# AbeelLab/phasm

Hardware: AMD Instinct MI355X
Metric: overlaps_per_sec (higher is better)
Workload: dtype u64

## Files before the change

phasm_amd/csrc/c_api.hip:

```cpp
#include "../../include/phasm_overlap.h"

#include <hip/hip_runtime.h>

#include <dlfcn.h>
#include <execinfo.h>
#include <fcntl.h>
#include <signal.h>
#include <sys/mman.h>
#include <sys/stat.h>
#include <unistd.h>

#include <algorithm>
#include <array>
#include <atomic>
#include <chrono>
#include <cmath>
#include <condition_variable>
#include <cstdio>
#include <cstdlib>
#include <cstring>
#include <deque>
#include <functional>
#include <memory>
#include <mutex>
// ... 526 lines not shown
}

bool kit_give(po_handle* h) {
    if (getenv("PHASM_NO_KIT_POOL") || !h->stream || !h->copy_stream || !h->up_stream || !h->rc_stream || !h->pinned) return false;
    if (hipStreamSynchronize(h->stream) != hipSuccess || hipStreamSynchronize(h->copy_stream) != hipSuccess ||
        hipStreamSynchronize(h->up_stream) != hipSuccess || hipStreamSynchronize(h->rc_stream) != hipSuccess) {
        (void)hipGetLastError();
        return false;
    }
    DevKit k;
    k.device = h->device;
    k.stream = h->stream;
    k.copy_stream = h->copy_stream;
    k.up_stream = h->up_stream;
    k.rc_stream = h->rc_stream;
    std::memcpy(k.ev_sets, h->ev_sets, sizeof(k.ev_sets));
    k.ev_up0 = h->ev_up0;
    k.ev_up1 = h->ev_up1;
    k.ev_meta = h->ev_meta;
    k.ev_first = h->ev_first;
    std::memcpy(k.ev_piece, h->ev_piece, sizeof(k.ev_piece));
    std::memcpy(k.ev_rc, h->ev_rc, sizeof(k.ev_rc));
    std::memcpy(k.ev_lay, h->ev_lay, sizeof(k.ev_lay));
    k.pinned = h->pinned;
    k.pinned_dev = h->pinned_dev;
    std::lock_guard<std::mutex> lock(g_kit_mu);
    if (g_kits.size() >= KIT_POOL_MAX) return false;
    g_kits.push_back(k);
    return true;
}


unsigned cpu_share() {
    static const unsigned share = [] {
        unsigned n = std::thread::hardware_concurrency();
        n = n ? n : 4u;
        long long q = -1, per = 100000;
        if (FILE* f = std::fopen("/sys/fs/cgroup/cpu.max", "r")) {
            char buf[64] = {0};
            if (std::fscanf(f, "%63s %lld", buf, &per) >= 1 && std::strcmp(buf, "max") != 0) q = atoll(buf);
            std::fclose(f);
        } else if (FILE* g = std::fopen("/sys/fs/cgroup/cpu/cpu.cfs_quota_us", "r")) {
            if (std::fscanf(g, "%lld", &q) != 1) q = -1;
            std::fclose(g);
            if (FILE* g2 = std::fopen("/sys/fs/cgroup/cpu/cpu.cfs_period_us", "r")) {
                if (std::fscanf(g2, "%lld", &per) != 1) per = 100000;
                std::fclose(g2);
            }
        }
        if (q > 0 && per > 0) n = std::min<unsigned>(n, (unsigned)std::max<long long>(1, q / per));
        return n;
    }();
    return share;
}

namespace home {

constexpr uint32_t CHUNK = 4096;

struct Job {
    const void* rec = nullptr;
    uint32_t sh_b = 0, sh_p = 0;
    uint64_t n_rec = 0;
    po_row* out = nullptr;
    uint64_t n_rows = 0;
    const volatile uint32_t* flag = nullptr;
    uint32_t want = 0;
    uint32_t paired = 0, bits = 2;
};

struct Pool {
    std::vector<std::thread> thr;
    std::mutex mu;
    std::condition_variable cv_queue;
    std::condition_variable cv_job;
    std::mutex call_mu;
    std::deque<Job> queue;
    std::atomic<uint64_t> submitted{0}, finished{0};
    std::atomic<int> error{0};
    const uint32_t* len = nullptr;
    uint32_t n_reads = 0;
    std::atomic<uint64_t> sum_l{0}, sum_b{0}, sum_e{0};
    Job cur;
    uint64_t job_seq = 0;
    uint32_t n_chunks = 0;
    std::vector<uint64_t> chunk_off;
    std::atomic<uint32_t> next_count{0}, done_count{0}, next_write{0}, done_write{0};
    std::atomic<int> phase{0};
    std::atomic<int> inside{0};
    std::chrono::steady_clock::time_point t0;
    std::vector<std::array<double, 3>> trace;
    bool tracing = false;
};

Pool* g_pool = nullptr;
std::once_flag g_pool_once;

inline void cpu_pause() {
#if defined(__x86_64__) || defined(__i386__)
    __builtin_ia32_pause();
#endif
}

std::atomic<uint32_t> g_spin_limit{4096};
template <class Pred>
inline void spin_until(Pred pred) {
    const uint32_t limit = g_spin_limit.load(std::memory_order_relaxed);
    for (uint32_t n = 0; !pred(); ++n) {
        if (limit == 0 || n < limit) cpu_pause();
        else std::this_thread::yield();
    }
}

inline po::Cand load_rec(const Job& j, uint64_t i) {
    if (!j.sh_b) return static_cast<const po::Cand*>(j.rec)[i];
    return po::unpack_record(static_cast<const uint64_t*>(j.rec)[i], j.sh_b, j.sh_p);
}

inline uint32_t rows_of_rec(const po::Cand& c, uint32_t paired) {
    if (!paired) return (c.type & 1u) + ((c.type >> 1) & 1u);
    return ((c.type & 1u) ? (c.a == (c.b ^ 1u) ? 1u : 2u) : 0u) + ((c.type & 2u) ? 2u : 0u);
}

inline void put_row(uint64_t*& o, uint32_t a, uint32_t b, uint32_t astart, uint32_t aend, uint32_t bend) {
    __builtin_nontemporal_store((uint64_t)a | ((uint64_t)b << 32), o);
    __builtin_nontemporal_store((uint64_t)astart | ((uint64_t)aend << 32), o + 1);
    __builtin_nontemporal_store((uint64_t)bend << 32, o + 2);
    o += 3;
}

bool expand_records(Pool& P, uint64_t lo, uint64_t hi, po_row* out) {
    uint64_t* o = reinterpret_cast<uint64_t*>(out);
    const Job& job = P.cur;
    const uint32_t* len = P.len;
    const uint32_t paired = job.paired, n_reads = P.n_reads, bits = job.bits;
    auto pb = [bits](uint32_t l) -> uint64_t { return bits == 8u ? l : (l >> 2) + ((l & 3u) != 0u); };
    uint64_t sl = 0, sb = 0, se = 0;
    for (uint64_t i = lo; i < hi; ++i) {
        const po::Cand c = load_rec(job, i);
        if (c.a >= n_reads || c.b >= n_reads) return false;
        const uint32_t la = len[c.a], lb = len[c.b];
        se += 2 * pb((c.type & 1u) ? la - c.p : lb);
        if (c.type & 1u) {
            const uint32_t l = la - c.p;
            const bool twin = paired && c.a != (c.b ^ 1u);
            put_row(o, c.a, c.b, c.p, la, l);
            if (twin) put_row(o, c.b ^ 1u, c.a ^ 1u, lb - l, lb, l);
            const uint64_t k = twin ? 2 : 1;
            sl += k * l;
            sb += k * 2 * pb(l);
        }
        if (c.type & 2u) {
            put_row(o, c.a, c.b, c.p, c.p + lb, lb);
            if (paired) put_row(o, c.a ^ 1u, c.b ^ 1u, la - c.p - lb, la - c.p, lb);
            const uint64_t k = paired ? 2 : 1;
            sl += k * lb;
            sb += k * 2 * pb(lb);
        }
    }
    P.sum_l.fetch_add(sl, std::memory_order_relaxed);
    P.sum_b.fetch_add(sb, std::memory_order_relaxed);
    P.sum_e.fetch_add(se, std::memory_order_relaxed);
    return true;
}

void run_phases(Pool& P, bool lead) {
    const uint32_t nc = P.n_chunks;
    for (;;) {
        const uint32_t c = P.next_count.fetch_add(1, std::memory_order_relaxed);
        if (c >= nc) break;
        const uint64_t lo = (uint64_t)c * CHUNK, hi = std::min<uint64_t>(P.cur.n_rec, lo + CHUNK);
        uint64_t n = 0;
        const uint32_t paired = P.cur.paired;
        for (uint64_t i = lo; i < hi; ++i) n += rows_of_rec(load_rec(P.cur, i), paired);
        P.chunk_off[c + 1] = n;
        P.done_count.fetch_add(1, std::memory_order_release);
    }
    if (lead) {
        spin_until([&] { return P.done_count.load(std::memory_order_acquire) >= nc; });
        P.chunk_off[0] = 0;
        for (uint32_t c = 0; c < nc; ++c) P.chunk_off[c + 1] += P.chunk_off[c];
        if (P.chunk_off[nc] != P.cur.n_rows) P.error.store(1);
        P.phase.store(P.error.load() ? 0 : 2, std::memory_order_release);
    } else {
        spin_until([&] { return P.phase.load(std::memory_order_acquire) != 1; });
    }
    if (P.phase.load(std::memory_order_acquire) != 2) return;
    for (;;) {
        const uint32_t c = P.next_write.fetch_add(1, std::memory_order_relaxed);
        if (c >= nc) break;
        const uint64_t lo = (uint64_t)c * CHUNK, hi = std::min<uint64_t>(P.cur.n_rec, lo + CHUNK);
        if (!expand_records(P, lo, hi, P.cur.out + P.chunk_off[c])) P.error.store(2);
#if defined(__x86_64__)
        __builtin_ia32_sfence();
#endif
        P.done_write.fetch_add(1, std::memory_order_release);
    }
}

void helper(Pool* Pp) {
    Pool& P = *Pp;
    uint64_t seen = 0;
    for (;;) {
        {
            std::unique_lock<std::mutex> lock(P.mu);
            P.cv_job.wait(lock, [&] { return P.job_seq != seen; });
            seen = P.job_seq;
        }
        P.inside.fetch_add(1, std::memory_order_acq_rel);
        if (P.phase.load(std::memory_order_acquire) != 0) run_phases(P, false);
        P.inside.fetch_sub(1, std::memory_order_release);
    }
}

void leader(Pool* Pp) {
    Pool& P = *Pp;
    for (;;) {
        Job j;
        {
            std::unique_lock<std::mutex> lock(P.mu);
            P.cv_queue.wait(lock, [&] { return !P.queue.empty(); });
            j = P.queue.front();
            P.queue.pop_front();
        }
        if (j.flag)
            spin_until([&] { return *j.flag == j.want; });
        std::atomic_thread_fence(std::memory_order_acquire);
        const double t_ready = P.tracing ? std::chrono::duration<double, std::micro>(std::chrono::steady_clock::now() - P.t0).count() : 0.0;
        if (P.error.load() == 0 && j.n_rec) {
            spin_until([&] { return P.inside.load(std::memory_order_acquire) == 0; });
            P.cur = j;
            P.n_chunks = (uint32_t)((j.n_rec + CHUNK - 1) / CHUNK);
            if (P.chunk_off.size() < (size_t)P.n_chunks + 1) P.chunk_off.resize((size_t)P.n_chunks + 1);
            P.next_count.store(0);
            P.done_count.store(0);
            P.next_write.store(0);
            P.done_write.store(0);
            P.phase.store(1, std::memory_order_release);
            {
                std::lock_guard<std::mutex> lock(P.mu);
                ++P.job_seq;
            }
            P.cv_job.notify_all();
            run_phases(P, true);
            if (P.phase.load() == 2)
                spin_until([&] { return P.done_write.load(std::memory_order_acquire) >= P.n_chunks; });
            P.phase.store(0, std::memory_order_release);
            std::atomic_thread_fence(std::memory_order_seq_cst);
        }
        if (P.tracing)
            P.trace.push_back({t_ready, std::chrono::duration<double, std::micro>(std::chrono::steady_clock::now() - P.t0).count(), (double)j.n_rows});
        P.finished.fetch_add(1, std::memory_order_release);
    }
}

Pool* pool() {
    std::call_once(g_pool_once, [] {
        Pool* P = new Pool();
        unsigned n = cpu_share();
        n = std::max(1u, std::min(n * 3 / 4, 12u));
        if (const char* e = getenv("PHASM_HOME_THREADS")) n = (unsigned)std::max(1, std::min(64, atoi(e)));
        try {
            P->thr.emplace_back(leader, P);
            P->thr.back().detach();
            for (unsigned i = 1; i < n; ++i) {
                P->thr.emplace_back(helper, P);
                P->thr.back().detach();
            }
        } catch (const std::system_error&) {
        }
        if (P->thr.empty()) {
            delete P;
            P = nullptr;
        }
        g_pool = P;
    });
    return g_pool;
}

void begin(Pool* P, const uint32_t* len, uint32_t n_reads, bool tracing) {
    if (const char* e = getenv("PHASM_HOME_SPIN")) g_spin_limit.store((uint32_t)std::max(0, atoi(e)));
    else g_spin_limit.store(4096);
    P->len = len;
    P->n_reads = n_reads;
    P->error.store(0);
    P->submitted.store(0);
    P->finished.store(0);
    P->sum_l.store(0);
    P->sum_b.store(0);
    P->sum_e.store(0);
    P->tracing = tracing;
    P->trace.clear();
    P->t0 = std::chrono::steady_clock::now();
}

void submit(Pool* P, const Job& j) {
    {
        std::lock_guard<std::mutex> lock(P->mu);
        P->queue.push_back(j);
    }
    P->submitted.fetch_add(1, std::memory_order_release);
    P->cv_queue.notify_one();
}

void wait_all(Pool* P) {
    spin_until([&] { return P->finished.load(std::memory_order_acquire) >= P->submitted.load(std::memory_order_acquire); });
}

}

po_status init_device(po_handle* h) {
    if (h->dev_ready) {
        HIP_TRY(h, hipSetDevice(h->device));
        return PO_OK;
    }
    AllocTrace tr("init_device", 0);
    const auto ti0 = std::chrono::steady_clock::now();
    auto imark = [&](const char* what) {
        if (tr.on) std::fprintf(stderr, "[init] %s at %.1f ms\n", what, std::chrono::duration<double, std::milli>(std::chrono::steady_clock::now() - ti0).count());
    };
    int n = 0;
    hipError_t e = hipGetDeviceCount(&n);
    imark("runtime up (hipGetDeviceCount)");
    if (e != hipSuccess || n == 0)
        return fail(h, PO_ERR_HIP, "no HIP device available (libphasm_overlap has no CPU fallback)");
    if (h->device < 0 || h->device >= n) return fail(h, PO_ERR_INVALID, "device ordinal out of range");
    HIP_TRY(h, hipSetDevice(h->device));
    hipDeviceProp_t prop;
    HIP_TRY(h, hipGetDeviceProperties(&prop, h->device));
    h->n_cu = prop.multiProcessorCount > 0 ? prop.multiProcessorCount : 256;
    h->lds_max = prop.sharedMemPerBlock;
    if (const char* e = getenv("PHASM_POISON")) h->poison = (int)(strtol(e, nullptr, 0) & 0xFF);
    if (!getenv("PHASM_NO_KIT_POOL") && kit_take(h)) {
        h->ev = h->ev_sets[0];
        std::memset(h->pinned, 0, 1024);
        hipLaunchKernelGGL(po::k_fill_u32, dim3(1), dim3(64), 0, h->stream, reinterpret_cast<uint32_t*>(h->pinned_dev + 63), (uint64_t)1, 0u);
        (void)hipGetLastError();
        h->dev_ready = true;
        return PO_OK;
    }
    imark("device selected, properties read");
    HIP_TRY(h, hipStreamCreateWithFlags(&h->stream, hipStreamNonBlocking));
    imark("first stream made");
    for (int i = 0; i < 2 * EV_N; ++i) HIP_TRY(h, hipEventCreate(&h->ev_sets[i / EV_N][i % EV_N]));
    HIP_TRY(h, hipEventCreate(&h->ev_up0));
    HIP_TRY(h, hipEventCreate(&h->ev_up1));
    imark("first events made");
    HIP_TRY(h, hipHostMalloc(reinterpret_cast<void**>(&h->pinned), 1024, hipHostMallocDefault));
    pin_note(h->pinned, 1024, 1u);
    HIP_TRY(h, hipHostGetDevicePointer(reinterpret_cast<void**>(&h->pinned_dev), h->pinned, 0));
    imark("landing zone made");
    if (const char* e = getenv("PHASM_POISON")) h->poison = (int)(strtol(e, nullptr, 0) & 0xFF);
    HIP_TRY(h, hipStreamCreateWithFlags(&h->copy_stream, hipStreamNonBlocking));
    imark("copy stream made");
    HIP_TRY(h, hipStreamCreateWithFlags(&h->up_stream, hipStreamNonBlocking));
    HIP_TRY(h, hipStreamCreateWithFlags(&h->rc_stream, hipStreamNonBlocking));
    imark("other streams made");
    for (int k = 0; k < PO_MAX_PIECES; ++k) {
        HIP_TRY(h, hipEventCreate(&h->ev_piece[k]));
        HIP_TRY(h, hipEventCreateWithFlags(&h->ev_rc[k], hipEventDisableTiming));
    }
    HIP_TRY(h, hipEventCreateWithFlags(&h->ev_first, hipEventDisableTiming));
    HIP_TRY(h, hipEventCreateWithFlags(&h->ev_meta, hipEventDisableTiming));
    imark("streams and events made");
    hipLaunchKernelGGL(po::k_fill_u32, dim3(1), dim3(64), 0, h->stream, reinterpret_cast<uint32_t*>(h->pinned_dev + 63), (uint64_t)1, 0u);
    (void)hipGetLastError();
    imark("first launch queued (code object loaded)");
    if (!getenv("PHASM_NO_WARM")) {
        void* w = nullptr;
        if (hipMalloc(&w, 256) == hipSuccess) {
            uint32_t* wd = static_cast<uint32_t*>(w);
            (void)hipMemcpyAsync(wd, h->pinned + 62, 8, hipMemcpyHostToDevice, h->up_stream);
            hipLaunchKernelGGL(po::k_fill_u32, dim3(1), dim3(64), 0, h->up_stream, wd + 8, (uint64_t)1, 0u);
            (void)hipMemcpyAsync(wd + 16, h->pinned + 62, 8, hipMemcpyHostToDevice, h->stream);
            hipLaunchKernelGGL(po::k_fill_u32, dim3(1), dim3(64), 0, h->rc_stream, wd + 24, (uint64_t)1, 0u);
            hipLaunchKernelGGL(po::k_fill_u32, dim3(1), dim3(64), 0, h->copy_stream, wd + 32, (uint64_t)1, 0u);
            (void)hipMemcpyAsync(h->pinned + 61, wd + 32, 8, hipMemcpyDeviceToHost, h->copy_stream);
// ... 3123 lines not shown
    *out = nullptr;
    if (h->segments_only) return fail(h, PO_ERR_INVALID, "this handle holds GFA segments without sequences");
    po_result* r = new (std::nothrow) po_result();
    if (!r) return fail(h, PO_ERR_NOMEM, "out of host memory");
    r->h = h;
    po_status st;
    try {
        st = upload(h);
        if (st == PO_OK) st = run_expand(h, candidates_device, n_candidates, r);
    } catch (const std::bad_alloc&) {
        st = fail(h, PO_ERR_NOMEM, "out of host memory in po_expand");
    }
    if (st != PO_OK) {
        if (h->dev_ready) (void)hipStreamSynchronize(h->stream);
        r->d_rows.release();
        delete r;
        return st;
    }
    ++h->live_results;
    *out = r;
    return PO_OK;
}

po_status po_overlaps(po_handle* h, uint32_t min_length, po_result** out) {
    return po_overlaps_shard(h, min_length, 0, 1, out);
}

extern "C++" {
namespace {

struct HostRows {
    HostBuf hb;
    uint64_t total = 0;
};

bool home_begin(po_handle* h) {
    h->home_on = false;
    if (!home_enabled()) return false;
    home::Pool* P = home::pool();
    if (!P) return false;
    P->call_mu.lock();
    home::begin(P, h->len.data(), (uint32_t)h->len.size(), getenv("PHASM_STREAM_TRACE") != nullptr || getenv("PHASM_HOME_TRACE") != nullptr);
    h->home_on = true;
    h->home_used = 0;
    h->home_seq = 0;
    if (h->home_pack_n != h->len.size() || h->home_pack_bases != h->total_bases) {
        uint32_t longest = 0;
        for (uint32_t l : h->len) longest = std::max(longest, l);
        uint32_t br = 1, bp = 1;
        while ((1ull << br) < (uint64_t)h->len.size()) ++br;
        while ((1ull << bp) < (uint64_t)longest + 1ull) ++bp;
        const bool fits = 2 * br + bp <= 62;
        h->home_pack_b = fits ? br : 0u;
        h->home_pack_p = fits ? 2 * br : 0u;
        h->home_pack_n = h->len.size();
        h->home_pack_bases = h->total_bases;
    }
    const char* pk = getenv("PHASM_HOME_PACK");
    const bool pack = !(pk && atoi(pk) == 0);
    h->home_sh_b = pack ? h->home_pack_b : 0u;
    h->home_sh_p = pack ? h->home_pack_p : 0u;
    return true;
}

void home_wait(po_handle* h) {
    if (h->home_on) home::wait_all(home::g_pool);
}

int home_end(po_handle* h, po_stats* sum = nullptr) {
    if (!h->home_on) return 0;
    home::Pool* P = home::g_pool;
    home::wait_all(P);
    const int err = P->error.load();
    if (sum) {
        sum->sum_overlap_bases += P->sum_l.load();
        sum->verify_bytes_algo += P->sum_b.load();
        sum->verify_bytes_exec += P->sum_e.load();
    }
    if (P->tracing)
        for (size_t i = 0; i < P->trace.size(); ++i)
            std::fprintf(stderr, "[home] piece %zu: records home at %.3f ms, %.0f rows written at %.3f ms (since the call set the pool up)\n", i,
                         P->trace[i][0] * 1e-3, P->trace[i][2], P->trace[i][1] * 1e-3);
    h->home_on = false;
    P->call_mu.unlock();
    return err;
}

po_status rows_room(po_handle* h, HostRows& R, uint64_t nk, uint32_t k, uint32_t n_chunks, double seen_share) {
    const size_t need = (size_t)(R.total + nk) * sizeof(po_row);
    if (need <= R.hb.cap) return PO_OK;
    uint64_t guess = std::max<uint64_t>(h->last_host_rows, (R.total + nk) * n_chunks / (k + 1));
    if (seen_share > 0.0) guess = std::max<uint64_t>(guess, (uint64_t)((double)(R.total + nk) / seen_share * 1.05));
    HostBuf bigger;
    PO_TRY(ensure_host(h, bigger, std::max<size_t>(need, (size_t)(guess + guess / 8) * sizeof(po_row))));
    home_wait(h);
    if (hipStreamSynchronize(h->copy_stream) != hipSuccess) {
        bigger.release();
        return fail(h, PO_ERR_HIP, "copy stream");
    }
    if (R.total) std::memcpy(bigger.p, R.hb.p, (size_t)R.total * sizeof(po_row));
    R.hb.release();
    R.hb = bigger;
    return PO_OK;
}

po_status append_home(po_handle* h, HostRows& R, const DevBuf& dev, uint64_t n_rec, uint64_t nk, uint32_t k, uint32_t n_chunks,
                      double seen_share = 0.0) {
    if (nk == 0) return PO_OK;
    home::Pool* P = home::g_pool;
    PO_TRY(rows_room(h, R, nk, k, n_chunks, seen_share));
    const size_t elem = h->home_sh_b ? sizeof(uint64_t) : sizeof(po::Cand);
    const size_t bytes = (size_t)n_rec * elem;
    constexpr uint64_t N_EV = 32;
    if (h->home_used + bytes > h->home_stage.cap || (h->home_seq && h->home_seq % N_EV == 0)) {
        home_wait(h);
        if (hipStreamSynchronize(h->copy_stream) != hipSuccess) return fail(h, PO_ERR_HIP, "copy stream");
        h->home_used = 0;
        if (bytes > h->home_stage.cap)
            PO_TRY(ensure_host(h, h->home_stage, std::max<size_t>({bytes * 2, (size_t)(h->home_last_bytes + h->home_last_bytes / 8), (size_t)8 << 20})));
    }
    const uint32_t slot = (uint32_t)(h->home_seq % N_EV);
    const uint32_t want = ++h->home_gen;
    char* dst = static_cast<char*>(h->home_stage.p) + h->home_used;
    HIP_TRY(h, hipMemcpyAsync(dst, dev.p, bytes, hipMemcpyDeviceToHost, h->copy_stream));
    hipLaunchKernelGGL(po::k_fill_u32, dim3(1), dim3(64), 0, h->copy_stream, reinterpret_cast<uint32_t*>(h->pinned_dev + 96 + slot), (uint64_t)1, want);
    HIP_TRY(h, hipGetLastError());
    home::Job j;
    j.rec = dst;
    j.sh_b = h->home_sh_b;
    j.sh_p = h->home_sh_p;
    j.n_rec = n_rec;
    j.out = static_cast<po_row*>(R.hb.p) + R.total;
    j.n_rows = nk;
    j.flag = reinterpret_cast<const volatile uint32_t*>(h->pinned + 96 + slot);
    j.want = want;
    j.paired = (h->bits == 2 && h->paired) ? 1u : 0u;
    j.bits = (uint32_t)h->bits;
    home::submit(P, j);
    ++h->home_seq;
    h->home_used += (bytes + 255) & ~size_t(255);
    h->home_last_bytes += bytes;
    R.total += nk;
    return PO_OK;
}

po_status append_rows(po_handle* h, HostRows& R, const DevBuf& dev, uint64_t nk, uint32_t k, uint32_t n_chunks, double seen_share = 0.0) {
    if (nk == 0) return PO_OK;
    PO_TRY(rows_room(h, R, nk, k, n_chunks, seen_share));
    HIP_TRY(h, hipMemcpyAsync(static_cast<char*>(R.hb.p) + (size_t)R.total * sizeof(po_row), dev.p, (size_t)nk * sizeof(po_row),
                              hipMemcpyDeviceToHost, h->copy_stream));
    R.total += nk;
    return PO_OK;
}

void add_stats(po_stats& sum, const po_stats& S) {
    sum.n_candidates += S.n_candidates;
    sum.n_verified += S.n_verified;
    sum.n_rows += S.n_rows;
    sum.sum_overlap_bases += S.sum_overlap_bases;
    sum.verify_bytes_algo += S.verify_bytes_algo;
    sum.verify_bytes_exec += S.verify_bytes_exec;
    sum.n_tiles += S.n_tiles;
    sum.shard_bases += S.shard_bases;
    sum.fused_tail += S.fused_tail;
    sum.tail_fallback += S.tail_fallback;
    sum.n_predicted += S.n_predicted;
// ... 1205 lines not shown
po_status po_result_merged_paths(po_result* r, uint64_t* n_paths, uint64_t* n_members, uint64_t* offsets_out, uint64_t cap_paths,
                                 uint32_t* members_out, int32_t* prefix_out, uint64_t cap_members, int64_t* lengths_out) {
    if (!r || !n_paths || !n_members) return PO_ERR_INVALID;
    *n_paths = *n_members = 0;
    po_handle* h = r->h;
    if (!h) return PO_ERR_INVALID;
    if (!r->merged) return fail(h, PO_ERR_INVALID, "po_result_merged_paths needs a po_layout_merge result");
    const uint64_t K = r->n_merged, m = r->n_members;
    *n_paths = K;
    *n_members = m;
    try {
        (void)hipSetDevice(h->device);
        HIP_TRY(h, hipStreamSynchronize(h->stream));
        if (offsets_out && cap_paths >= K) {
            std::vector<uint32_t> off(K);
            if (K) HIP_TRY(h, hipMemcpy(off.data(), r->d_moff.p, K * 4, hipMemcpyDeviceToHost));
            for (uint64_t k = 0; k < K; ++k) offsets_out[k] = off[k];
            offsets_out[K] = m;
        }
        if (lengths_out && cap_paths >= K && K) HIP_TRY(h, hipMemcpy(lengths_out, r->d_mlen.p, K * 8, hipMemcpyDeviceToHost));
        if (members_out && cap_members >= m && m) HIP_TRY(h, hipMemcpy(members_out, r->d_member.p, m * 4, hipMemcpyDeviceToHost));
        if (prefix_out && cap_members >= m && m) HIP_TRY(h, hipMemcpy(prefix_out, r->d_prefix.p, m * 4, hipMemcpyDeviceToHost));
    } catch (const std::bad_alloc&) {
        return fail(h, PO_ERR_NOMEM, "out of host memory in po_result_merged_paths");
    }
    return PO_OK;
}

po_status po_result_node_order(po_result* r, uint32_t* nodes_out, uint64_t cap, uint64_t* n_out) {
    if (!r || !n_out || (!nodes_out && cap)) return PO_ERR_INVALID;
    *n_out = 0;
    po_handle* h = r->h;
    if (!h) return PO_ERR_INVALID;
    if (!r->kind_edges || !r->d_nrank.p) return fail(h, PO_ERR_INVALID, "po_result_node_order needs an edge result");
    const size_t n_nodes = h->len.size() + (r->merged ? (size_t)r->n_merged : 0);
    try {
        std::vector<unsigned long long> rank(n_nodes);
        (void)hipSetDevice(h->device);
        HIP_TRY(h, hipStreamSynchronize(h->stream));
        if (n_nodes) HIP_TRY(h, hipMemcpy(rank.data(), r->d_nrank.p, n_nodes * 8, hipMemcpyDeviceToHost));
        std::vector<std::pair<unsigned long long, uint32_t>> order;
        for (size_t i = 0; i < n_nodes; ++i)
            if (rank[i] != po::NODE_NO_RANK) order.emplace_back(rank[i], (uint32_t)i);
        std::sort(order.begin(), order.end());
        *n_out = order.size();
        for (size_t i = 0; i < order.size() && i < cap; ++i) nodes_out[i] = order[i].second;
    } catch (const std::bad_alloc&) {
        return fail(h, PO_ERR_NOMEM, "out of host memory in po_result_node_order");
    }
    return PO_OK;
}

uint64_t po_debug_host_ranges(uint64_t* out, uint64_t cap_entries) {
    std::lock_guard<std::mutex> lock(g_pin_mu);
    const uint64_t n = std::min<uint64_t>(cap_entries, g_pins.size());
    for (uint64_t i = 0; out && i < n; ++i) {
        out[3 * i] = g_pins[i].base;
        out[3 * i + 1] = g_pins[i].bytes;
        out[3 * i + 2] = g_pins[i].kind;
    }
    return g_pins.size();
}

uint64_t po_debug_store_words(const po_handle* h, int store, const uint64_t** words) {
    if (!h || store < 0 || store > 1) return 0;
    if (words) *words = h->words[store].data();
    return h->words[store].size();
}

int po_debug_expand_records(const po_cand* records, uint64_t n, const uint32_t* lengths, uint32_t n_reads, uint32_t paired,
                            po_row* rows_out, uint64_t n_rows_expected) {
    home::Pool* P = home::pool();
    if (!P) return -1;
    std::lock_guard<std::mutex> call(P->call_mu);
    home::begin(P, lengths, n_reads, false);
    home::Job j;
    j.rec = records;
    j.n_rec = n;
    j.out = rows_out;
    j.n_rows = n_rows_expected;
    j.paired = paired ? 1u : 0u;
    home::submit(P, j);
    home::wait_all(P);
    return P->error.load();
}

int po_debug_expand_packed(const uint64_t* records, uint64_t n, uint32_t sh_b, uint32_t sh_p, const uint32_t* lengths, uint32_t n_reads,
                           uint32_t paired, po_row* rows_out, uint64_t n_rows_expected) {
    if (!sh_b || sh_p < sh_b || sh_p >= 62) return -2;
    home::Pool* P = home::pool();
    if (!P) return -1;
    std::lock_guard<std::mutex> call(P->call_mu);
    home::begin(P, lengths, n_reads, false);
    home::Job j;
    j.rec = records;
    j.sh_b = sh_b;
    j.sh_p = sh_p;
    j.n_rec = n;
    j.out = rows_out;
    j.n_rows = n_rows_expected;
    j.paired = paired ? 1u : 0u;
    home::submit(P, j);
    home::wait_all(P);
    return P->error.load();
}

static int g_fault_fd = 2;
static struct sigaction g_fault_prev[2];
static void fault_handler(int sig, siginfo_t* si, void* ctx) {
    char line[128];
    const int n = std::snprintf(line, sizeof(line), "[phasm] signal %d at address %p (code %d); native stack of the faulting thread:\n", sig,
                                si ? si->si_addr : nullptr, si ? si->si_code : 0);
    if (n > 0) (void)!::write(g_fault_fd, line, (size_t)n);
    void* frames[64];
    const int k = backtrace(frames, 64);
    backtrace_symbols_fd(frames, k, g_fault_fd);
    const struct sigaction& prev = g_fault_prev[sig == SIGBUS ? 1 : 0];
    if ((prev.sa_flags & SA_SIGINFO) && prev.sa_sigaction) {
        prev.sa_sigaction(sig, si, ctx);
        return;
    }
    if (prev.sa_handler != SIG_DFL && prev.sa_handler != SIG_IGN && prev.sa_handler) {
        prev.sa_handler(sig);
        return;
    }
    signal(sig, SIG_DFL);
    raise(sig);
}

int po_debug_fault_backtrace(int fd) {
    g_fault_fd = fd;
    struct sigaction sa;
    std::memset(&sa, 0, sizeof(sa));
    sa.sa_sigaction = fault_handler;
    sa.sa_flags = SA_SIGINFO | SA_NODEFER;
    sigemptyset(&sa.sa_mask);
    void* warm[4];
    (void)backtrace(warm, 4);
    return (sigaction(SIGSEGV, &sa, &g_fault_prev[0]) == 0 && sigaction(SIGBUS, &sa, &g_fault_prev[1]) == 0) ? 0 : -1;
}

int po_debug_pointer_info(const void* p, int32_t* hip_type, int32_t* hsa_type, uint64_t* base, uint64_t* bytes) {
    if (hip_type) *hip_type = -1;
    if (hsa_type) *hsa_type = -1;
    if (base) *base = 0;
    if (bytes) *bytes = 0;
    if (!p) return 0;
    int known = 0;
    {
        hipPointerAttribute_t at;
        std::memset(&at, 0, sizeof(at));
        const hipError_t e = hipPointerGetAttributes(&at, p);
        if (e == hipSuccess) {
            if (hip_type) *hip_type = (int32_t)at.type;
            if (at.type != hipMemoryTypeUnregistered) known = 1;
        } else {
            (void)hipGetLastError();
        }
    }
    {
        struct PtrInfo {
            uint32_t size;
            uint32_t type;
            void* agentBaseAddress;
            void* hostBaseAddress;
            size_t sizeInBytes;
            void* userData;
            uint64_t agentOwner;
            uint32_t global_flags;
        };
        using Fn = int (*)(const void*, PtrInfo*, void* (*)(size_t), uint32_t*, void**);
        static Fn fn = reinterpret_cast<Fn>(dlsym(RTLD_DEFAULT, "hsa_amd_pointer_info"));
        if (fn) {
            PtrInfo info;
            std::memset(&info, 0, sizeof(info));
            info.size = sizeof(info);
            if (fn(p, &info, nullptr, nullptr, nullptr) == 0) {
                if (hsa_type) *hsa_type = (int32_t)info.type;
                if (info.type != 0) {
                    known = 1;
                    if (base) *base = (uint64_t)(uintptr_t)(info.hostBaseAddress ? info.hostBaseAddress : info.agentBaseAddress);
                    if (bytes) *bytes = info.sizeInBytes;
                }
            }
        }
    }
// ... 13 lines not shown
```

phasm_amd/csrc/kernels.hip.h:

```cpp
#pragma once
#include <hip/hip_runtime.h>
#include <stdint.h>

namespace po {

using u32x4 = __attribute__((ext_vector_type(4))) uint32_t;

constexpr uint32_t NO_SELFREP = 0xFFFFFFFFu;
constexpr uint64_t KEY_EMPTY = ~0ull;
constexpr int WAVE = 64;

#ifndef PO_VER_PAD
#define PO_VER_PAD 0
#endif
#ifndef PO_SCAN_PAD
#define PO_SCAN_PAD 0
#endif
template <int N>
__device__ __forceinline__ void valu_pad(uint32_t& r, uint32_t c) {
#pragma unroll
    for (int i = 0; i < N; ++i) asm volatile("v_xor_b32 %0, %0, %1" : "+v"(r) : "v"(c));
}

struct CandGuard {
// ... 711 lines not shown
        uint32_t T[48];
        auto make_T = [&](int s) __attribute__((always_inline)) {
            const int j = (2 * s) >> 5, sh = (2 * s) & 31;
            T[s] = sh ? __builtin_amdgcn_alignbit(x[j + 1], x[j], sh) : x[j];
        };
        typedef uint32_t __attribute__((ext_vector_type(2))) u32x2;
        typedef const u32x2 __attribute__((address_space(3))) lds_u32x2;
        auto block_of = [&](int s) __attribute__((always_inline)) -> u32x2 {
            const uint32_t addr = FULLK ? (T[s + 1] & amask) : (((T[s] & klo) >> 2) & amask);
            return *reinterpret_cast<lds_u32x2*>((uintptr_t)addr);
        };
        static_assert(PO_FILTER_DEPTH >= 1 && PO_FILTER_DEPTH <= 16, "the T window below reaches 17 bases ahead");
        u32x2 blk[PO_FILTER_DEPTH];
#pragma unroll
        for (int s = 0; s <= 16; ++s) make_T(s);
#pragma unroll
        for (int s = 0; s < PO_FILTER_DEPTH; ++s) blk[s] = block_of(s);
        __builtin_amdgcn_sched_barrier(0);
#pragma unroll
        for (int s = 0; s < 32; ++s) {
            if (s + 17 < 48) make_T(s + 17);
            const uint32_t t1 = T[s] & klo, t2 = T[s + 16] & khi;
            const uint32_t sel2 = FULLK ? T[s + 10] : (t1 >> 20);
            const u32x2 b = blk[s % PO_FILTER_DEPTH];
            hitmask = __builtin_amdgcn_alignbit((b.x >> (t1 & 31)) & (b.x >> (sel2 & 31)) & (b.y >> (t2 & 31)), hitmask, 1);
            if (s + PO_FILTER_DEPTH < 32) blk[s % PO_FILTER_DEPTH] = block_of(s + PO_FILTER_DEPTH);
            if constexpr (PO_SCAN_PAD > 0) valu_pad<PO_SCAN_PAD>(hitmask, 0u);
            asm volatile("" : "+v"(hitmask));
            __builtin_amdgcn_sched_barrier(0);
        }
    } else {
        const uint32_t wshift = 32 - (bloom_log2 - 5);
#pragma unroll
        for (int s = 0; s < W; ++s) {
            const uint64_t kmer = FULLK ? window<BITS>(w0, w1, s) : (window<BITS>(w0, w1, s) & kmask);
            const uint32_t lo = (uint32_t)kmer, hi = (uint32_t)(kmer >> 32);
            const uint32_t h1 = (lo ^ ((hi << 13) | (hi >> 19))) * 0x9E3779B1u;
            const uint32_t bm = (1u << ((h1 >> 7) & 31)) | (1u << ((h1 >> 12) & 31)) | (1u << ((h1 >> 2) & 31));
            const uint32_t bw = s_bloom[h1 >> wshift];
            hitmask |= ((bw & bm) == bm ? 1u : 0u) << s;
        }
    }
    return hitmask;
}

template <bool STREAM = false, typename F>
__device__ inline void for_each_candidate(const uint32_t* __restrict__ chain, const uint32_t* __restrict__ len,
                                          uint32_t paired, uint32_t z, uint32_t w, uint32_t a, uint32_t rem, F&& f) {
    if (w & SLOT_SINGLE) {
        const uint32_t lb = w & ~SLOT_SINGLE;
        const uint32_t k = keep_bits<STREAM>(a, z, rem, lb, paired);
        if (k) f(z, lb, k);
    } else {
        for (uint32_t j = 0; j < w; ++j) {
            const uint32_t b = chain[z + j];
            const uint32_t lb = len[b];
            const uint32_t k = keep_bits<STREAM>(a, b, rem, lb, paired);
            if (k) f(b, lb, k);
        }
    }
}

#ifndef PO_LEFT_CAP
#define PO_LEFT_CAP 2048
#endif
constexpr uint32_t LEFT_CAP = PO_LEFT_CAP;
constexpr int SCAN_LDS_PER_WAVE = 2 * WAVE * 4 + WAVE * 4;
#ifdef PO_STAMPS
#define PO_STAMP(var) do { __builtin_amdgcn_sched_barrier(0); asm volatile("s_memtime %0\n\ts_waitcnt lgkmcnt(0)" : "=s"(var) :: "memory"); __builtin_amdgcn_sched_barrier(0); } while (0)
#else
#define PO_STAMP(var) do { } while (0)
#endif

template <int BITS, bool FULLK, bool STREAM = false>
__global__ __launch_bounds__(SCAN_BLOCK) void k_scan_probe(const ScanArgs A) {
    constexpr int W = 64 / BITS;
    extern __shared__ uint64_t smem[];
    const uint32_t nwaves = blockDim.x >> 6;
    const uint32_t lane = lane_id(), wave = threadIdx.x >> 6;
    const uint32_t bloom_words = (1u << A.bloom_log2) >> 5;
    uint32_t* s_bloom = reinterpret_cast<uint32_t*>(smem);
    uint32_t* qs = s_bloom + bloom_words + wave * (2 * WAVE);
    uint32_t* tm = s_bloom + bloom_words + (2 * nwaves + wave) * WAVE;
    for (uint32_t i = threadIdx.x; i < bloom_words; i += blockDim.x) s_bloom[i] = A.bloom[i];
    tm[lane] = 0;
    __syncthreads();

    const uint32_t stride = gridDim.x * nwaves;
    const uint32_t tbits = A.tbits, tmask = (1u << A.tbits) - 1u;
    const Slot* __restrict__ table = A.table;
    const uint32_t* __restrict__ chain = A.chain;
    const uint32_t* __restrict__ len = A.len;
    const uint64_t* __restrict__ words = A.words;
    const TileRec* __restrict__ tiles = A.tiles;
    uint32_t* __restrict__ selfrep = A.selfrep;
    uint32_t* __restrict__ n_selfrep = A.n_selfrep;
    uint32_t* __restrict__ truemask = A.truemask;
    uint32_t* __restrict__ tile_count = A.tile_count;
    const uint32_t paired = A.paired, m = A.m, tile_end = A.tile_end;
    const uint64_t kmask = A.kmask;

    uint64_t pk = 0;
    u32x4 ps0 = {0, 0, 0, 0}, ps1 = {0, 0, 0, 0}, ps2 = {0, 0, 0, 0}, ps3 = {0, 0, 0, 0};
    uint32_t pidx = 0, psrc = 0;
    bool pon = false;
    uint64_t pk2 = 0;
    u32x4 pt0 = {0, 0, 0, 0}, pt1 = {0, 0, 0, 0}, pt2 = {0, 0, 0, 0}, pt3 = {0, 0, 0, 0};
    uint32_t pidx2 = 0, psrc2 = 0;
    bool pon2 = false, extra = false;
    uint32_t prev_t = 0xFFFFFFFFu, prev_a = 0, prev_la = 0, prev_word0 = 0;

    auto count_slot = [&](u32x4 s, uint32_t a, uint32_t la, uint32_t p) __attribute__((always_inline)) -> uint32_t {
        uint32_t n = 0;
        if (p > 0) {
            if (s.w & SLOT_SINGLE) {
                if (s.z == a) note_selfrep(selfrep, a, p, n_selfrep);
            } else {
                for (uint32_t j = 0; j < s.w; ++j)
                    if (chain[s.z + j] == a) note_selfrep(selfrep, a, p, n_selfrep);
            }
        }
        for_each_candidate<STREAM>(chain, len, paired, s.z, s.w, a, la - p, [&](uint32_t, uint32_t, uint32_t) { ++n; });
        return n;
    };
    uint2* __restrict__ my_left = A.left + (size_t)(blockIdx.x * nwaves + wave) * LEFT_CAP;
    uint32_t left_n = 0;
    auto defer = [&](bool want, uint32_t tile, uint32_t lane_s) __attribute__((always_inline)) -> bool {
        const uint64_t bal = __ballot(want);
        if (bal == 0) return false;
        const uint32_t cnt = (uint32_t)__popcll(bal);
        if (left_n + cnt > LEFT_CAP) return false;
        if (want) my_left[left_n + (uint32_t)__popcll(bal & ((1ull << lane) - 1ull))] = uint2{tile, lane_s};
        left_n = __builtin_amdgcn_readfirstlane(left_n + cnt);
        return want;
    };

    const uint32_t t_last = tile_end - 1;
    uint32_t t = __builtin_amdgcn_readfirstlane(A.tile_begin + blockIdx.x * nwaves + wave);
    if (t >= tile_end) return;
    auto ld16 = [](const void* ptr) __attribute__((always_inline)) -> u32x4 {
        u32x4 v;
        asm volatile("global_load_dwordx4 %0, %1, off" : "=v"(v) : "v"(ptr) : "memory");
        return v;
    };
    TileRec rec = tiles[t];
    u32x4 r_lo, r_hi, wa, wb = {0, 0, 0, 0};
    {
        const TileRec* rp = &tiles[__builtin_amdgcn_readfirstlane(min(t + stride, t_last))];
        r_lo = ld16(rp);
        r_hi = ld16(reinterpret_cast<const char*>(rp) + 16);
        wa = ld16(&words[rec.wabs + lane]);
        ps0 = ld16(&table[0]);
        ps1 = ld16(&table[1]);
        ps2 = ld16(&table[2]);
        ps3 = ld16(&table[3]);
    }
#ifdef PO_STAMPS
    unsigned long long acc_s[6] = {0, 0, 0, 0, 0, 0};
#endif
    auto pass = [&](u32x4& wcur, u32x4& wnext) __attribute__((always_inline)) -> bool {
        const bool have_tile = t < tile_end;
        const uint32_t tn = t + stride;
        unsigned long long st0 = 0, st1 = 0, st2 = 0, st3 = 0, st4 = 0, st5 = 0;
        (void)st0; (void)st1; (void)st2; (void)st3; (void)st4; (void)st5;
        PO_STAMP(st0);
        asm volatile("s_cmp_eq_u32 %3, 0\n\ts_cbranch_scc1 .Lpo_w4_%=\n\ts_waitcnt vmcnt(8)\n\ts_branch .Lpo_wd_%=\n"
                     ".Lpo_w4_%=:\n\ts_waitcnt vmcnt(4)\n.Lpo_wd_%=:"
// ... 1736 lines not shown
```

Before: 1.581 billion.

## Spin-wait pool helpers during calls and vectorize bloom filter LDS staging

After: 1.577 billion. About the same (-0.3%).

```diff
diff --git a/phasm_amd/csrc/c_api.hip b/phasm_amd/csrc/c_api.hip
--- a/phasm_amd/csrc/c_api.hip
+++ b/phasm_amd/csrc/c_api.hip
@@ -632,7 +632,8 @@
     uint32_t n_reads = 0;
     std::atomic<uint64_t> sum_l{0}, sum_b{0}, sum_e{0};
     Job cur;
-    uint64_t job_seq = 0;
+    std::atomic<uint64_t> job_seq{0};
+    std::atomic<bool> in_call{false};
     uint32_t n_chunks = 0;
     std::vector<uint64_t> chunk_off;
     std::atomic<uint32_t> next_count{0}, done_count{0}, next_write{0}, done_write{0};
@@ -752,10 +753,16 @@
     Pool& P = *Pp;
     uint64_t seen = 0;
     for (;;) {
+        if (P.in_call.load(std::memory_order_acquire)) {
+            const uint32_t limit = g_spin_limit.load(std::memory_order_relaxed);
+            for (uint32_t n = 0; (limit == 0 || n < limit) && P.job_seq.load(std::memory_order_acquire) == seen &&
+                                 P.in_call.load(std::memory_order_relaxed); ++n)
+                cpu_pause();
+        }
         {
             std::unique_lock<std::mutex> lock(P.mu);
-            P.cv_job.wait(lock, [&] { return P.job_seq != seen; });
-            seen = P.job_seq;
+            P.cv_job.wait(lock, [&] { return P.job_seq.load(std::memory_order_relaxed) != seen; });
+            seen = P.job_seq.load(std::memory_order_relaxed);
         }
         P.inside.fetch_add(1, std::memory_order_acq_rel);
         if (P.phase.load(std::memory_order_acquire) != 0) run_phases(P, false);
@@ -789,7 +796,7 @@
             P.phase.store(1, std::memory_order_release);
             {
                 std::lock_guard<std::mutex> lock(P.mu);
-                ++P.job_seq;
+                P.job_seq.fetch_add(1, std::memory_order_release);
             }
             P.cv_job.notify_all();
             run_phases(P, true);
@@ -842,7 +849,10 @@
     P->tracing = tracing;
     P->trace.clear();
     P->t0 = std::chrono::steady_clock::now();
-}
+    P->in_call.store(true, std::memory_order_release);
+}
+
+void end(Pool* P) { P->in_call.store(false, std::memory_order_release); }
 
 void submit(Pool* P, const Job& j) {
     {
@@ -4132,6 +4142,7 @@
             std::fprintf(stderr, "[home] piece %zu: records home at %.3f ms, %.0f rows written at %.3f ms (since the call set the pool up)\n", i,
                          P->trace[i][0] * 1e-3, P->trace[i][2], P->trace[i][1] * 1e-3);
     h->home_on = false;
+    home::end(P);
     P->call_mu.unlock();
     return err;
 }
@@ -5503,6 +5514,7 @@
     j.paired = paired ? 1u : 0u;
     home::submit(P, j);
     home::wait_all(P);
+    home::end(P);
     return P->error.load();
 }
 
@@ -5523,6 +5535,7 @@
     j.paired = paired ? 1u : 0u;
     home::submit(P, j);
     home::wait_all(P);
+    home::end(P);
     return P->error.load();
 }
 
diff --git a/phasm_amd/csrc/kernels.hip.h b/phasm_amd/csrc/kernels.hip.h
--- a/phasm_amd/csrc/kernels.hip.h
+++ b/phasm_amd/csrc/kernels.hip.h
@@ -817,7 +817,25 @@
     uint32_t* s_bloom = reinterpret_cast<uint32_t*>(smem);
     uint32_t* qs = s_bloom + bloom_words + wave * (2 * WAVE);
     uint32_t* tm = s_bloom + bloom_words + (2 * nwaves + wave) * WAVE;
-    for (uint32_t i = threadIdx.x; i < bloom_words; i += blockDim.x) s_bloom[i] = A.bloom[i];
+    {
+        const uint32_t last = (bloom_words >> 2) - 1u, bd = blockDim.x;
+        const u32x4* __restrict__ gv = reinterpret_cast<const u32x4*>(A.bloom);
+        u32x4* sv = reinterpret_cast<u32x4*>(s_bloom);
+        for (uint32_t base = threadIdx.x; base <= last; base += 8 * bd) {
+            const uint32_t i0 = base, i1 = min(base + bd, last), i2 = min(base + 2 * bd, last), i3 = min(base + 3 * bd, last),
+                           i4 = min(base + 4 * bd, last), i5 = min(base + 5 * bd, last), i6 = min(base + 6 * bd, last),
+                           i7 = min(base + 7 * bd, last);
+            const u32x4 v0 = gv[i0], v1 = gv[i1], v2 = gv[i2], v3 = gv[i3], v4 = gv[i4], v5 = gv[i5], v6 = gv[i6], v7 = gv[i7];
+            sv[i0] = v0;
+            sv[i1] = v1;
+            sv[i2] = v2;
+            sv[i3] = v3;
+            sv[i4] = v4;
+            sv[i5] = v5;
+            sv[i6] = v6;
+            sv[i7] = v7;
+        }
+    }
     tm[lane] = 0;
     __syncthreads();
 
```
